# LeoIV/polyaxon

Measured on AMD Instinct MI355X. Metric: HPO trials/hour (whole node) + wall-clock-to-target, ResNet-50 Hyperband sweep, higher is better.
Workload: dtype bf16

## Files before the change

polyaxon_amd/csrc/bn_kernels.hip:

```cpp
#include <hip/hip_runtime.h>

#include "handoff.h"
#include <stdint.h>

#define PLX_API extern "C" __attribute__((visibility("default")))

namespace {

constexpr int kBlock = 256;

struct alignas(16) bf16x8 {
  uint16_t v[8];
};

__device__ __forceinline__ float bf2f(uint16_t b) { return __uint_as_float(((uint32_t)b) << 16); }

__device__ __forceinline__ uint16_t f2bf(float f) {
  return __builtin_bit_cast(uint16_t, (__bf16)f);
}

__device__ __forceinline__ void load8(const bf16x8* p, float* f) {
  const bf16x8 v = *p;
#pragma unroll
  for (int k = 0; k < 8; ++k) f[k] = bf2f(v.v[k]);
// ... 554 lines not shown
inline void reduce_finalize_fwd(hipStream_t stream, const float* part, int nblk, float* l2, unsigned* cnt,
                                const FwdFin& f) {
  const int C = f.C, S = (nblk + kRowsPerSplit - 1) / kRowsPerSplit;
  if (cnt != nullptr) {
    hipLaunchKernelGGL(bn_fwd_reduce_finalize_kernel<kFinNT>, dim3((C + 63) / 64, S), dim3(kFinNT), 0, stream, part, nblk, l2, S,
                       cnt, f);
    return;
  }
  hipLaunchKernelGGL(bn_partial_reduce_kernel<kFinNT>,
                     dim3((C + 63) / 64, S, 2), dim3(kFinNT), 0, stream, part, nblk, C, l2, S);
  hipLaunchKernelGGL(bn_fwd_finalize_kernel<kFinNT>, dim3((C + 63) / 64),
                     dim3(kFinNT), 0, stream, l2, l2 + (int64_t)S * C, S,
                     f.x_row0, C, f.M, f.gamma, f.beta, f.eps, f.momentum, f.running_mean, f.running_var, f.save_mean,
                     f.save_invstd, f.scale, f.bias);
}

inline void reduce_finalize_bwd(hipStream_t stream, const float* part, int nblk, float* l2, unsigned* cnt,
                                const BwdFin& f) {
  const int C = f.C, S = (nblk + kRowsPerSplit - 1) / kRowsPerSplit;
  if (cnt != nullptr) {
    hipLaunchKernelGGL(bn_bwd_reduce_finalize_kernel<kFinNT>, dim3((C + 63) / 64, S), dim3(kFinNT), 0, stream, part, nblk, l2, S,
                       cnt, f);
    return;
  }
  hipLaunchKernelGGL(bn_partial_reduce_kernel<kFinNT>,
                     dim3((C + 63) / 64, S, 2), dim3(kFinNT), 0, stream, part, nblk, C, l2, S);
  hipLaunchKernelGGL(bn_bwd_finalize_kernel<kFinNT>, dim3((C + 63) / 64),
                     dim3(kFinNT), 0, stream, l2, l2 + (int64_t)S * C, S, C,
                     f.M, f.gamma, f.mean, f.invstd, f.dgamma, f.dbeta, f.coef, f.accumulate);
}

struct alignas(8) u8x8 {
  uint8_t v[8];
};

__global__ __launch_bounds__(256) void stem_apply_pool_kernel(const bf16x8* __restrict__ x,
                                                              const float* __restrict__ sb, bf16x8* __restrict__ y,
                                                              u8x8* __restrict__ idx, int N, int H, int W, int G,
                                                              int OH, int OW) {
  const unsigned j = blockIdx.x * 256u + threadIdx.x;
  if (j >= (unsigned)(OW * G)) return;
  const unsigned g = j % (unsigned)G, ow = j / (unsigned)G;
  const int C = G * 8;
  float a[8], b[8];
#pragma unroll
  for (int k = 0; k < 8; ++k) {
    a[k] = sb[g * 8 + k];
    b[k] = sb[C + g * 8 + k];
  }
  for (int row = blockIdx.y; row < N * OH; row += gridDim.y) {
    const int n = row / OH, oh = row - n * OH;
    float best[8];
    uint8_t arg[8];
#pragma unroll
    for (int k = 0; k < 8; ++k) {
      best[k] = -INFINITY;
      arg[k] = 255;
    }
    uint4 q[9];
    bool ok[9];
#pragma unroll
    for (int kh = 0; kh < 3; ++kh) {
      const int ih = oh * 2 - 1 + kh;
      const int ihc = ih < 0 ? 0 : (ih >= H ? H - 1 : ih);
#pragma unroll
      for (int kw = 0; kw < 3; ++kw) {
        const int iw = (int)ow * 2 - 1 + kw;
        const int iwc = iw < 0 ? 0 : (iw >= W ? W - 1 : iw);
        ok[kh * 3 + kw] = ih >= 0 && ih < H && iw >= 0 && iw < W;
        q[kh * 3 + kw] = *(const uint4*)(x + ((size_t)(n * H + ihc) * W + iwc) * G + g);
      }
    }
#pragma unroll
    for (int t9 = 0; t9 < 9; ++t9) {
      const uint32_t qw[4] = {q[t9].x, q[t9].y, q[t9].z, q[t9].w};
#pragma unroll
      for (int k = 0; k < 8; ++k) {
        const float xk = __uint_as_float((k & 1) ? (qw[k >> 1] & 0xffff0000u) : (qw[k >> 1] << 16));
        const float f = (float)(__bf16)fmaxf(fmaf(xk, a[k], b[k]), 0.f);
        if (ok[t9] && (f > best[k] || arg[k] == 255)) {
          best[k] = f;
          arg[k] = (uint8_t)t9;
        }
      }
    }
    bf16x8 o;
    u8x8 m;
#pragma unroll
    for (int k = 0; k < 8; ++k) {
      o.v[k] = f2bf(best[k]);
      m.v[k] = arg[k];
    }
    const size_t t = (size_t)row * OW * G + j;
    y[t] = o;
    idx[t] = m;
  }
}

__device__ __forceinline__ int stem_cover(int i, int O, int* o, int* k) {
  int n = 0;
  if (i & 1) {
    if ((i + 1) >> 1 < O) { o[n] = (i + 1) >> 1; k[n++] = 0; }
    o[n] = (i - 1) >> 1; k[n++] = 2;
  } else if ((i >> 1) < O) {
    o[n] = i >> 1; k[n++] = 1;
  }
  return n;
}

template <bool DX>
__global__ __launch_bounds__(256) void stem_pool_bn_bwd_kernel(const bf16x8* __restrict__ dy, const u8x8* __restrict__ idx,
                                                               const bf16x8* __restrict__ x, const float* __restrict__ sb,
                                                               const float* __restrict__ mean,
                                                               const float* __restrict__ invstd,
                                                               const float* __restrict__ coef, bf16x8* __restrict__ dx,
                                                               float* __restrict__ part, int N, int H, int W, int G,
                                                               int OH, int OW) {
  const int QH = (H + 1) / 2, QW = (W + 1) / 2;
  const unsigned j0 = blockIdx.x * 256u + threadIdx.x;
  const bool active = j0 < (unsigned)(QW * G);
  const unsigned j = active ? j0 : 0u;
  const unsigned g = j % (unsigned)G;
  const int qb = (int)(j / (unsigned)G);
  const int C = G * 8;
  float a[8], b[8], c1[8], c2[8], c3[8], s1[8], s2[8];
#pragma unroll
  for (int k = 0; k < 8; ++k) {
    a[k] = sb[g * 8 + k];
    b[k] = sb[C + g * 8 + k];
    if constexpr (DX) {
      c1[k] = coef[g * 8 + k];
      c2[k] = coef[C + g * 8 + k];
      c3[k] = coef[2 * C + g * 8 + k];
    } else {
      c1[k] = mean[g * 8 + k];
      c2[k] = invstd[g * 8 + k];
      c3[k] = 0.f;
    }
    s1[k] = s2[k] = 0.f;
  }
  for (int row = blockIdx.y; active && row < N * QH; row += gridDim.y) {
    const int n = row / QH, qa = row - n * QH;
    uint2 am[4];
    uint4 d[4], xq[4];
    bool wv[4], pv[4];
#pragma unroll
    for (int p = 0; p < 2; ++p)
#pragma unroll
      for (int q = 0; q < 2; ++q) {
        const int w4 = p * 2 + q, oh = qa + p, ow = qb + q;
        wv[w4] = oh < OH && ow < OW;
        const size_t off = ((size_t)(n * OH + (oh < OH ? oh : OH - 1)) * OW + (ow < OW ? ow : OW - 1)) * G + g;
        am[w4] = *(const uint2*)(idx + off);
        d[w4] = *(const uint4*)(dy + off);
        if (!wv[w4]) am[w4] = make_uint2(0xffffffffu, 0xffffffffu);
        const int ih = 2 * qa + p, iw = 2 * qb + q;
        pv[w4] = ih < H && iw < W;
        xq[w4] = *(const uint4*)(x + ((size_t)(n * H + (ih < H ? ih : H - 1)) * W + (iw < W ? iw : W - 1)) * G + g);
      }
#pragma unroll
    for (int di = 0; di < 2; ++di)
#pragma unroll
      for (int dj = 0; dj < 2; ++dj) {
        const int e = di * 2 + dj;
        const uint32_t xw[4] = {xq[e].x, xq[e].y, xq[e].z, xq[e].w};
        float o[8];
#pragma unroll
        for (int k = 0; k < 8; ++k) {
          float acc = 0.f;
#pragma unroll
          for (int p = 0; p < 2; ++p)
#pragma unroll
            for (int q = 0; q < 2; ++q) {
              const int kh = di + 1 - 2 * p, kw = dj + 1 - 2 * q;
              if (kh < 0 || kw < 0) continue;
              const int w4 = p * 2 + q;
              const uint32_t ab = (k < 4 ? am[w4].x : am[w4].y) >> (8 * (k & 3)) & 0xffu;
              const uint32_t dw = (k >> 1) == 0 ? d[w4].x : (k >> 1) == 1 ? d[w4].y : (k >> 1) == 2 ? d[w4].z : d[w4].w;
              const float dv = __uint_as_float((k & 1) ? (dw & 0xffff0000u) : (dw << 16));
              acc += ab == (uint32_t)(kh * 3 + kw) ? dv : 0.f;
            }
          const float xf = __uint_as_float((k & 1) ? (xw[k >> 1] & 0xffff0000u) : (xw[k >> 1] << 16));
          const float dz = (pv[e] && fmaf(xf, a[k], b[k]) > 0.f) ? (float)(__bf16)acc : 0.f;
          if constexpr (DX) {
            o[k] = fmaf(c1[k], dz, fmaf(c2[k], xf, c3[k]));
          } else {
            s1[k] += dz;
            s2[k] = fmaf(dz, (xf - c1[k]) * c2[k], s2[k]);
          }
        }
        if constexpr (DX) {
          if (pv[e]) store8(dx + ((size_t)(n * H + 2 * qa + di) * W + 2 * qb + dj) * G + g, o);
        }
      }
  }
  if constexpr (!DX) {
    __shared__ float red[256 * 17];
#pragma unroll
    for (int k = 0; k < 8; ++k) {
      red[threadIdx.x * 17 + k] = s1[k];
      red[threadIdx.x * 17 + 8 + k] = s2[k];
    }
    __syncthreads();
    const int nb = gridDim.x * gridDim.y, blk = blockIdx.y * gridDim.x + blockIdx.x;
    for (int e = threadIdx.x; e < G * 16; e += 256) {
      const int gg = e % G, v = e / G;
      float sum = 0.f;
      for (int r = gg; r < 256; r += G) sum += red[r * 17 + v];
      const int c = gg * 8 + (v & 7);
      part[((int64_t)(v < 8 ? 0 : nb) + blk) * C + c] = sum;
    }
  }
}

constexpr int g_stem_bwd_cap = 4096;

inline dim3 stem_bwd_grid(int N, int H, int W, int G, bool dx) {
  const int rows = N * ((H + 1) / 2), cap = dx ? 65535 : g_stem_bwd_cap;
  return dim3((((W + 1) / 2) * G + 255) / 256, rows < cap ? rows : cap);
}

}

PLX_API int64_t plx_bn_workspace(int64_t M, int C) {
  Plan p;
  if (!plan_for(M, C, &p)) return -1;
  return 2 * (int64_t)(p.nblk + p.S) * C;
}

PLX_API int plx_bn_forward(const void* x, const void* res, void* y, int64_t M, int C, const float* gamma,
                           const float* beta, float eps, float momentum, float* running_mean, float* running_var,
                           float* save_mean, float* save_invstd, float* scale_bias ,
                           float* partials , uint8_t* mask ,
                           int relu, const float* res_sb ,
                           unsigned* counters ,
                           hipStream_t stream) {
  Plan p;
  if (!plan_for(M, C, &p) || M < 1) return 1;
  float* psum = partials;
  float* psq = partials + (int64_t)p.nblk * C;
  hipLaunchKernelGGL(bn_stats_kernel, dim3(p.nblk, p.gy), dim3(kBlock), 0, stream, (const bf16x8*)x, M, p.G, p.Gb,
                     p.rows_per_block, psum, psq);
  float* l2 = partials + 2 * (int64_t)p.nblk * C;
  reduce_finalize_fwd(stream, partials, p.nblk, l2, counters,
                      FwdFin{(const uint16_t*)x, C, M, gamma, beta, eps, momentum, running_mean, running_var,
                             save_mean, save_invstd, scale_bias, scale_bias + C});
  const int64_t n_vec = M * p.G;
  if (y != nullptr)
    launch_apply(stream, n_vec, p.G, x, res, y, scale_bias, scale_bias + C, relu, relu ? mask : nullptr, res_sb);
  return (int)hipGetLastError();
}

PLX_API int64_t plx_bn_l2_workspace(int nblk, int C) {
  return 2 * (int64_t)((nblk + kRowsPerSplit - 1) / kRowsPerSplit) * C;
}

PLX_API int plx_bn_forward_from_partials(const void* x, const void* res, void* y, int64_t M, int C,
                                         const float* gamma, const float* beta, float eps, float momentum,
                                         float* running_mean, float* running_var, float* save_mean,
                                         float* save_invstd, float* scale_bias, const float* partials, int nblk,
                                         float* l2, uint8_t* mask, int relu, const float* res_sb,
                                         unsigned* counters, hipStream_t stream) {
  Plan p;
  if (!plan_for(M, C, &p) || M < 1 || nblk < 1) return 1;
  reduce_finalize_fwd(stream, partials, nblk, l2, counters,
                      FwdFin{nullptr, C, M, gamma, beta, eps, momentum, running_mean, running_var, save_mean,
                             save_invstd, scale_bias, scale_bias + C});
  const int64_t n_vec = M * p.G;
  if (y != nullptr)
    launch_apply(stream, n_vec, p.G, x, res, y, scale_bias, scale_bias + C, relu, relu ? mask : nullptr, res_sb);
  return (int)hipGetLastError();
}

PLX_API int plx_bn_apply(const void* x, const void* res, void* y, int64_t M, int C, const float* scale_bias, int relu,
                         hipStream_t stream) {
  Plan p;
  if (!plan_for(M, C, &p)) return 1;
  const int64_t n_vec = M * p.G;
  launch_apply(stream, n_vec, p.G, x, res, y, scale_bias, scale_bias + C, relu, nullptr, nullptr);
  return (int)hipGetLastError();
}

PLX_API int plx_bn_apply_res_relu(const void* x, const void* res, void* y, int64_t M, int C, const float* scale_bias,
                                  uint8_t* mask, const float* res_sb, hipStream_t stream) {
  Plan p;
  if (!plan_for(M, C, &p) || M < 1 || res == nullptr || mask == nullptr) return 1;
  launch_apply(stream, M * p.G, p.G, x, res, y, scale_bias, scale_bias + C, 1, mask, res_sb);
  return (int)hipGetLastError();
}

PLX_API int plx_bn_dx_blocks(int64_t M, int C) {
  Plan p;
  if (!plan_for(M, C, &p)) return -1;
  return apply_grid(M * p.G, p.G);
}

PLX_API int plx_bn_backward(const void* x, const uint8_t* mask, const void* dy, void* dx, void* dres, int64_t M, int C,
                            const float* gamma, const float* save_mean, const float* save_invstd, float* dgamma,
                            float* dbeta, float* coef , float* partials , int relu,
                            int accumulate, const ResBn* resbn , unsigned* counters,
                            hipStream_t stream) {
  Plan p;
  if (!plan_for(M, C, &p) || M < 1 || (relu && mask == nullptr)) return 1;
  if (resbn != nullptr && (dres == nullptr || resbn->part == nullptr)) return 1;
  const ResBn rb = resbn != nullptr ? *resbn : ResBn{};
  float* pa = partials;
  float* pb = partials + (int64_t)p.nblk * C;
  hipLaunchKernelGGL(relu ? bn_bwd_reduce_kernel<true> : bn_bwd_reduce_kernel<false>, dim3(p.nblk, p.gy), dim3(kBlock), 0, stream, (const bf16x8*)x,
                     mask, (const bf16x8*)dy, M, p.G, p.Gb, p.rows_per_block, save_mean, save_invstd,
                     relu, pa, pb);
  float* l2 = partials + 2 * (int64_t)p.nblk * C;
  reduce_finalize_bwd(stream, partials, p.nblk, l2, counters,
                      BwdFin{C, M, gamma, save_mean, save_invstd, dgamma, dbeta, coef, accumulate});
  const int64_t n_vec = M * p.G;
  launch_dx(stream, n_vec, p.G, x, mask, dy, dx, dres, coef, relu, rb);
  return (int)hipGetLastError();
}

PLX_API int plx_bn_backward_from_partials(const void* x, const uint8_t* mask, const void* dy, void* dx, void* dres,
                                          int64_t M, int C, const float* gamma, const float* save_mean,
                                          const float* save_invstd, float* dgamma, float* dbeta, float* coef,
                                          const float* partials, int nblk, float* l2, int relu, int accumulate,
                                          const ResBn* resbn, unsigned* counters, hipStream_t stream) {
  Plan p;
  if (!plan_for(M, C, &p) || M < 1 || nblk < 1 || (relu && mask == nullptr)) return 1;
  if (resbn != nullptr && (dres == nullptr || resbn->part == nullptr)) return 1;
  const ResBn rb = resbn != nullptr ? *resbn : ResBn{};
  reduce_finalize_bwd(stream, partials, nblk, l2, counters,
                      BwdFin{C, M, gamma, save_mean, save_invstd, dgamma, dbeta, coef, accumulate});
  const int64_t n_vec = M * p.G;
  launch_dx(stream, n_vec, p.G, x, mask, dy, dx, dres, coef, relu, rb);
  return (int)hipGetLastError();
}

PLX_API int plx_bn_backward_coef(const void* x, const uint8_t* mask, const void* dy, int64_t M, int C,
                                 const float* gamma, const float* save_mean, const float* save_invstd, float* dgamma,
                                 float* dbeta, float* coef, float* partials, int relu, int accumulate,
                                 unsigned* counters, hipStream_t stream) {
  Plan p;
  if (!plan_for(M, C, &p) || M < 1 || (relu && mask == nullptr)) return 1;
  float* pa = partials;
  float* pb = partials + (int64_t)p.nblk * C;
  hipLaunchKernelGGL(relu ? bn_bwd_reduce_kernel<true> : bn_bwd_reduce_kernel<false>, dim3(p.nblk, p.gy), dim3(kBlock), 0, stream, (const bf16x8*)x,
                     mask, (const bf16x8*)dy, M, p.G, p.Gb, p.rows_per_block, save_mean, save_invstd,
                     relu, pa, pb);
  reduce_finalize_bwd(stream, partials, p.nblk, partials + 2 * (int64_t)p.nblk * C, counters,
                      BwdFin{C, M, gamma, save_mean, save_invstd, dgamma, dbeta, coef, accumulate});
  return (int)hipGetLastError();
}

PLX_API int plx_bn_backward_coef_from_partials(int64_t M, int C, const float* gamma, const float* save_mean,
                                               const float* save_invstd, float* dgamma, float* dbeta, float* coef,
                                               const float* partials, int nblk, float* l2, int accumulate,
                                               unsigned* counters, hipStream_t stream) {
  Plan p;
  if (!plan_for(M, C, &p) || M < 1 || nblk < 1) return 1;
  reduce_finalize_bwd(stream, partials, nblk, l2, counters,
                      BwdFin{C, M, gamma, save_mean, save_invstd, dgamma, dbeta, coef, accumulate});
  return (int)hipGetLastError();
}

PLX_API int plx_stem_bn_pool_forward(const void* x, void* y, void* idx, int N, int H, int W, int C, const float* gamma,
                                     const float* beta, float eps, float momentum, float* running_mean,
                                     float* running_var, float* save_mean, float* save_invstd, float* scale_bias,
                                     float* partials, const float* ext_part, int ext_nblk, unsigned* counters,
                                     hipStream_t stream) {
  const int G = C / 8;
  if (N <= 0 || H <= 0 || W <= 0 || C % 8 || G > 256 || 256 % G) return 1;
  const int rc = ext_part != nullptr
                     ? plx_bn_forward_from_partials(x, nullptr, nullptr, (int64_t)N * H * W, C, gamma, beta, eps,
                                                    momentum, running_mean, running_var, save_mean, save_invstd,
                                                    scale_bias, ext_part, ext_nblk, partials, nullptr, 1, nullptr,
                                                    counters, stream)
                     : plx_bn_forward(x, nullptr, nullptr, (int64_t)N * H * W, C, gamma, beta, eps, momentum,
                                      running_mean, running_var, save_mean, save_invstd, scale_bias, partials, nullptr,
                                      1, nullptr, counters, stream);
  if (rc) return rc;
  const int OH = (H - 1) / 2 + 1, OW = (W - 1) / 2 + 1;
  const int rows = N * OH;
  hipLaunchKernelGGL(stem_apply_pool_kernel, dim3((OW * G + 255) / 256, rows < 65535 ? rows : 65535), dim3(256), 0,
                     stream, (const bf16x8*)x, scale_bias, (bf16x8*)y, (u8x8*)idx, N, H, W, G, OH, OW);
  return (int)hipGetLastError();
}


PLX_API int64_t plx_stem_bn_pool_bwd_workspace(int N, int H, int W, int C) {
  const dim3 g = stem_bwd_grid(N, H, W, C / 8, false);
  const int64_t nblk = (int64_t)g.x * g.y;
  return 2 * (nblk + (nblk + kRowsPerSplit - 1) / kRowsPerSplit) * C;
}

PLX_API int plx_stem_bn_pool_backward(const void* dy, const void* idx, const void* x, void* dx, int N, int H, int W,
                                      int C, const float* gamma, const float* save_mean, const float* save_invstd,
                                      const float* scale_bias, float* dgamma, float* dbeta, float* coef,
                                      float* workspace, int accumulate, unsigned* counters, hipStream_t stream) {
  const int G = C / 8;
  if (N <= 0 || H <= 0 || W <= 0 || C % 8 || G > 256 || 256 % G) return 1;
  const int OH = (H - 1) / 2 + 1, OW = (W - 1) / 2 + 1;
  const dim3 grid = stem_bwd_grid(N, H, W, G, false), grid_dx = stem_bwd_grid(N, H, W, G, true);
  const int nblk = grid.x * grid.y;
  hipLaunchKernelGGL(stem_pool_bn_bwd_kernel<false>, grid, dim3(256), 0, stream, (const bf16x8*)dy, (const u8x8*)idx,
                     (const bf16x8*)x, scale_bias, save_mean, save_invstd, (const float*)nullptr, (bf16x8*)nullptr,
                     workspace, N, H, W, G, OH, OW);
  reduce_finalize_bwd(stream, workspace, nblk, workspace + 2 * (int64_t)nblk * C, counters,
                      BwdFin{C, (int64_t)N * H * W, gamma, save_mean, save_invstd, dgamma, dbeta, coef, accumulate});
  hipLaunchKernelGGL(stem_pool_bn_bwd_kernel<true>, grid_dx, dim3(256), 0, stream, (const bf16x8*)dy, (const u8x8*)idx,
                     (const bf16x8*)x, scale_bias, save_mean, save_invstd, coef, (bf16x8*)dx, (float*)nullptr, N, H,
                     W, G, OH, OW);
  return (int)hipGetLastError();
}
```

polyaxon_amd/ops/bn_fused.py:

```python
from __future__ import annotations

import ctypes

from typing import Optional

import torch

from polyaxon_amd.ops import _native
from polyaxon_amd.ops.conv1x1 import BnLink, PendingApply, fill_pending
from polyaxon_amd.ops.flat import direct_grad


def _stream() -> int:
    return _native.current_stream()


_COUNTERS = {}


def _counters(dev: torch.device):
    key = (dev.index, torch.cuda.current_stream(dev).cuda_stream)
    return _native.cached(_COUNTERS, key, lambda: torch.zeros(64, dtype=torch.int32, device=dev)).data_ptr()


def _cl(t: torch.Tensor) -> torch.Tensor:
    return t if t.is_contiguous(memory_format=torch.channels_last) else t.contiguous(memory_format=torch.channels_last)


def supported(x: torch.Tensor) -> bool:
    if not x.is_cuda or x.dtype != torch.bfloat16 or x.dim() != 4:
        return False
    c = x.shape[1]
    g = c // 8
    return c % 8 == 0 and g > 0 and (g & (g - 1)) == 0 and x.numel() > 0


class _BNAct(torch.autograd.Function):
    @staticmethod
    def forward(ctx, x, weight, bias, running_mean, running_var, residual, momentum, eps, relu, ext=None, box=None,
                link=None, rlink=None, defer=False, dxsink=None, pend=None):
        lib = _native.lib("plx_bn")
        ctx.dxsink = dxsink if x.is_contiguous(memory_format=torch.channels_last) else None
        x = _cl(x)
        n, c, h, w = x.shape
        m = n * h * w
        ws = _native.size("plx_bn", "plx_bn_workspace", m, c)
        if ws < 0:
            raise RuntimeError("unsupported channel count for fused BN")
        f32 = dict(dtype=torch.float32, device=x.device)
        defer = bool(defer) and not relu and residual is None and link is not None
        y = None if defer else torch.empty_like(x, memory_format=torch.channels_last)
        holder, pend = pend, pend is not None and relu and residual is not None and not defer
        yp = y.data_ptr() if (y is not None and not pend) else None
        stats = torch.empty(4 * c, **f32)
        res_sb = None
        if residual is not None:
            rl = getattr(residual, "_plx_bn_link", None)
            if rl is not None and rl.affine is not None and getattr(residual, "_plx_deferred", False):
                res_sb = rl.affine
        res = _cl(residual) if residual is not None else None
        rsp = res_sb.data_ptr() if res_sb is not None else None
        rm = running_mean.data_ptr() if running_mean is not None else None
        rv = running_var.data_ptr() if running_var is not None else None
        mask = torch.empty(m * c // 8, dtype=torch.uint8, device=x.device) if relu else None
        mp = mask.data_ptr() if mask is not None else None
        if ext is not None:
            part, nblk = ext
            l2 = torch.empty(_native.size("plx_bn", "plx_bn_l2_workspace", nblk, c), **f32)
            rc = lib.plx_bn_forward_from_partials(
                x.data_ptr(), res.data_ptr() if res is not None else None, yp, m, c, weight.data_ptr(),
                bias.data_ptr(), float(eps), float(momentum), rm, rv, stats.data_ptr(), stats[c:].data_ptr(),
                stats[2 * c:].data_ptr(), part.data_ptr(), nblk, l2.data_ptr(), mp, int(relu), rsp,
                _counters(x.device), _stream())
            _native.check(rc, "plx_bn_forward_from_partials")
        else:
            partials = torch.empty(ws, **f32)
            rc = lib.plx_bn_forward(
                x.data_ptr(), res.data_ptr() if res is not None else None, yp, m, c,
                weight.data_ptr(), bias.data_ptr(), float(eps), float(momentum), rm, rv,
                stats.data_ptr(), stats[c:].data_ptr(), stats[2 * c:].data_ptr(), partials.data_ptr(), mp, int(relu),
                rsp, _counters(x.device), _stream())
            _native.check(rc, "plx_bn_forward")
        ctx.save_for_backward(x, mask, weight, stats)
        ctx.pending = PendingApply(x, res, stats[2 * c:], res_sb, mask, y) if pend else None
        if pend:
            holder.append(ctx.pending)
        ctx.relu = relu
        ctx.has_res = residual is not None
        ctx.box = box if (box is not None and box.armed and residual is not None) else None
        if ctx.box is not None:
            ctx.box.expect = True
        ctx.ws = ws
        gw, gb = direct_grad(weight), direct_grad(bias)
        ctx.direct = (gw, gb) if (gw is not None and gb is not None) else None
        ctx.link = link
        if link is not None:
            link.x, link.mask, link.mean, link.invstd = x, mask, stats[:c], stats[c:2 * c]
            if defer:
                link.affine = stats[2 * c:]
        ctx.rlink = rlink if (rlink is not None and residual is not None and rlink.x is not None
                              and rlink.x.shape == x.shape and ctx.box is None) else None
        if defer:
            return x.view_as(x)
        return y

    @staticmethod
    def backward(ctx, dy):
        lib = _native.lib("plx_bn")
        x, mask, weight, stats = ctx.saved_tensors
        if ctx.pending is not None:
            ctx.pending.check_done()
        n, c, h, w = x.shape
        m = n * h * w
        dy = _cl(dy)
        if dy.dtype != torch.bfloat16:
            dy = dy.to(torch.bfloat16)
        f32 = dict(dtype=torch.float32, device=x.device)
        dx = torch.empty_like(x, memory_format=torch.channels_last)
        masked_box = ctx.box is not None and ctx.relu and mask is not None
        dres = (torch.empty_like(x, memory_format=torch.channels_last)
                if ctx.has_res and not masked_box else None)
        if ctx.direct is not None:
            dg_ptr, db_ptr, acc = ctx.direct[0].data_ptr(), ctx.direct[1].data_ptr(), 1
            dgb = None
        else:
            dgb = torch.empty(2 * c, **f32)
            dg_ptr, db_ptr, acc = dgb.data_ptr(), dgb[c:].data_ptr(), 0
        coef = torch.empty(3 * c, **f32)
        part, nblk = ctx.link.take() if ctx.link is not None else (None, 0)
        if ctx.dxsink is not None and dres is None:
            if part is not None:
                l2 = torch.empty(_native.size("plx_bn", "plx_bn_l2_workspace", nblk, c), **f32)
                rc = lib.plx_bn_backward_coef_from_partials(
                    m, c, weight.data_ptr(), stats.data_ptr(), stats[c:].data_ptr(), dg_ptr, db_ptr, coef.data_ptr(),
                    part.data_ptr(), nblk, l2.data_ptr(), acc, _counters(x.device), _stream())
                _native.check(rc, "plx_bn_backward_coef_from_partials")
            else:
                partials = torch.empty(ctx.ws, **f32)
                rc = lib.plx_bn_backward_coef(
                    x.data_ptr(), mask.data_ptr() if mask is not None else None, dy.data_ptr(), m, c,
                    weight.data_ptr(), stats.data_ptr(), stats[c:].data_ptr(), dg_ptr, db_ptr, coef.data_ptr(),
                    partials.data_ptr(), int(ctx.relu), acc, _counters(x.device), _stream())
                _native.check(rc, "plx_bn_backward_coef")
            ctx.dxsink.put(dy, x, mask if ctx.relu else None, coef, dx)
            if ctx.box is not None:
                ctx.box.put_masked(dy, mask)
            dgamma = dgb[:c] if dgb is not None else None
            dbeta = dgb[c:] if dgb is not None else None
            return dx, dgamma, dbeta, None, None, None, None, None, None, None, None, None, None, None, None, None
        rb = None
        if ctx.rlink is not None and dres is not None:
            rl = ctx.rlink
            nblk2 = _native.size("plx_bn", "plx_bn_dx_blocks", m, c)
            rl.part = torch.empty(2 * nblk2 * c, **f32)
            rl.nblk = nblk2
            rb = _native.ResBnArgs(rl.x.data_ptr(), rl.mask.data_ptr() if rl.mask is not None else None,
                                   rl.mean.data_ptr(), rl.invstd.data_ptr(), rl.part.data_ptr())
        rbp = ctypes.addressof(rb) if rb is not None else None
        if part is not None:
            l2 = torch.empty(_native.size("plx_bn", "plx_bn_l2_workspace", nblk, c), **f32)
            rc = lib.plx_bn_backward_from_partials(
                x.data_ptr(), mask.data_ptr() if mask is not None else None, dy.data_ptr(), dx.data_ptr(),
                dres.data_ptr() if dres is not None else None, m, c, weight.data_ptr(), stats.data_ptr(),
                stats[c:].data_ptr(), dg_ptr, db_ptr, coef.data_ptr(), part.data_ptr(), nblk, l2.data_ptr(),
                int(ctx.relu), acc, rbp, _counters(x.device), _stream())
            _native.check(rc, "plx_bn_backward_from_partials")
        else:
            partials = torch.empty(ctx.ws, **f32)
            rc = lib.plx_bn_backward(
                x.data_ptr(), mask.data_ptr() if mask is not None else None, dy.data_ptr(), dx.data_ptr(),
                dres.data_ptr() if dres is not None else None, m, c, weight.data_ptr(), stats.data_ptr(),
                stats[c:].data_ptr(), dg_ptr, db_ptr, coef.data_ptr(), partials.data_ptr(), int(ctx.relu), acc,
                rbp, _counters(x.device), _stream())
            _native.check(rc, "plx_bn_backward")
        if ctx.box is not None:
            if masked_box:
                ctx.box.put_masked(dy, mask)
            else:
                ctx.box.put(dres)
            dres = None
        dgamma = dgb[:c] if dgb is not None else None
        dbeta = dgb[c:] if dgb is not None else None
        return dx, dgamma, dbeta, None, None, dres, None, None, None, None, None, None, None, None, None, None


class _Materialize(torch.autograd.Function):

    @staticmethod
    def forward(ctx, t, sb):
        c = t.shape[1]
        return (t.float() * sb[:c].view(1, c, 1, 1) + sb[c:].view(1, c, 1, 1)).to(t.dtype).contiguous(
            memory_format=torch.channels_last)

    @staticmethod
    def backward(ctx, g):
        return g, None


def materialize(t: Optional[torch.Tensor]) -> Optional[torch.Tensor]:
    if t is None:
        return t
    fill_pending(t)
    if not getattr(t, "_plx_deferred", False):
        return t
    return _Materialize.apply(t, t._plx_bn_link.affine)


def bn_act(x: torch.Tensor, weight: torch.Tensor, bias: torch.Tensor, running_mean: Optional[torch.Tensor],
           running_var: Optional[torch.Tensor], training: bool, momentum: float, eps: float,
           residual: Optional[torch.Tensor], act: bool, ext_stats=None, residual_grad_box=None,
           residual_link: bool = False, defer_apply: bool = False, dx_sink=None,
           defer_res_relu: bool = False) -> torch.Tensor:
    fill_pending(residual)
    if residual is not None and residual.dtype != x.dtype:
        residual = residual.to(x.dtype)
    if training:
        link = BnLink()
        rlink = getattr(residual, "_plx_bn_link", None) if (residual_link and residual is not None) else None
        defer = bool(defer_apply) and not act and residual is None
        pend = [] if (defer_res_relu and act and residual is not None) else None
        y = _BNAct.apply(x, weight, bias, running_mean, running_var, residual, momentum, eps, act, ext_stats,
                         residual_grad_box, link, rlink, defer, dx_sink, pend)
        y._plx_bn_link = link
        if defer:
            y._plx_deferred = True
        if pend:
            y._plx_pending = pend[0]
        return y
    residual = materialize(residual)
    lib = _native.lib("plx_bn")
    x = _cl(x)
    n, c, h, w = x.shape
    inv = torch.rsqrt(running_var.float() + eps)
    scale = weight.float() * inv
    sb = torch.cat([scale, bias.float() - running_mean.float() * scale]).contiguous()
    y = torch.empty_like(x, memory_format=torch.channels_last)
    res = _cl(residual) if residual is not None else None
    rc = lib.plx_bn_apply(x.data_ptr(), res.data_ptr() if res is not None else None, y.data_ptr(), n * h * w, c,
                          sb.data_ptr(), int(act), _stream())
    _native.check(rc, "plx_bn_apply")
    return y
```

polyaxon_amd/ops/conv1x1.py:

```python
from __future__ import annotations

import ctypes
import os
from typing import Dict

import torch
import torch.nn as nn
import torch.nn.functional as F

from polyaxon_amd.ops import _native, side_stream, wcache
from polyaxon_amd.ops.flat import direct_grad

_ZERO: Dict[int, torch.Tensor] = {}
_CUS: Dict[int, int] = {}

_BN_DX_FUSED = os.environ.get("PLX_BN_DX_FUSED", "1") != "0"


def set_bn_dx_fused(on: bool) -> bool:
    global _BN_DX_FUSED
    prev, _BN_DX_FUSED = _BN_DX_FUSED, bool(on)
    return prev


_BN_APPLY_FUSED = os.environ.get("PLX_BN_APPLY_FUSED", "1") != "0"


def set_bn_apply_fused(on: bool) -> bool:
    global _BN_APPLY_FUSED
    prev, _BN_APPLY_FUSED = _BN_APPLY_FUSED, bool(on)
    return prev


def bn_apply_fused() -> bool:
    return _BN_APPLY_FUSED


def _zero_page(dev: torch.device) -> torch.Tensor:
    idx = dev.index if dev.index is not None else torch.cuda.current_device()
    return _native.cached(_ZERO, idx, lambda: torch.zeros(256, dtype=torch.bfloat16, device=dev))


def _num_cus(dev: torch.device) -> int:
    idx = dev.index if dev.index is not None else torch.cuda.current_device()
    if idx not in _CUS:
        _CUS[idx] = torch.cuda.get_device_properties(idx).multi_processor_count
    return _CUS[idx]


def _stream() -> int:
    return _native.current_stream()


def nt_stats_rows(n: int) -> int:
    return _native.size("plx_conv", "plx_gemm_nt_rows_per_block", n)


def gemm_nt(a: torch.Tensor, b: torch.Tensor, out: torch.Tensor = None, stats: torch.Tensor = None,
            add: torch.Tensor = None, bnr: "_native.BnBwdArgs" = None, add_mask: torch.Tensor = None) -> torch.Tensor:
    m, k = a.shape
    n = b.shape[0]
    if out is None:
        out = torch.empty(m, n, dtype=torch.bfloat16, device=a.device)
    assert a.stride(1) == 1 and b.stride(1) == 1 and out.stride(1) == 1 and b.shape[1] == k
    assert a.data_ptr() % 16 == 0 and b.data_ptr() % 16 == 0 and out.data_ptr() % 16 == 0
    if stats is not None:
        nblk = -(-m // nt_stats_rows(n))
        assert stats.dtype == torch.float32 and stats.is_contiguous() and stats.numel() >= 2 * nblk * n
    if add is not None:
        assert add.shape == (m, n) and add.stride(1) == 1 and add.dtype == torch.bfloat16 and add.data_ptr() % 16 == 0
    if add_mask is not None:
        assert add is not None and add.stride(0) == n and add_mask.dtype == torch.uint8 and add_mask.numel() == m * n // 8
    rc = _native.lib("plx_conv").plx_gemm_nt(a.data_ptr(), b.data_ptr(), out.data_ptr(), m, n, k, a.stride(0),
                                             b.stride(0), out.stride(0), _zero_page(a.device).data_ptr(),
                                             stats.data_ptr() if stats is not None else None,
                                             add.data_ptr() if add is not None else None,
                                             add.stride(0) if add is not None else 0,
                                             add_mask.data_ptr() if add_mask is not None else None,
                                             ctypes.addressof(bnr) if bnr is not None else None, _stream())
    _native.check(rc, "plx_gemm_nt")
    return out


def gemm_nt_bndx(g: torch.Tensor, x: torch.Tensor, mask: torch.Tensor, coef: torch.Tensor, dy: torch.Tensor,
                 b: torch.Tensor, out: torch.Tensor = None, add: torch.Tensor = None,
                 bnr: "_native.BnBwdArgs" = None, add_mask: torch.Tensor = None) -> torch.Tensor:
    m, k = g.shape
    n = b.shape[0]
    if out is None:
        out = torch.empty(m, n, dtype=torch.bfloat16, device=g.device)
    for t in (g, x, dy):
        assert t.shape == (m, k) and t.dtype == torch.bfloat16 and t.stride() == (k, 1) and t.data_ptr() % 16 == 0
    assert b.stride(1) == 1 and out.stride(1) == 1 and b.shape[1] == k and b.dtype == torch.bfloat16
    assert b.data_ptr() % 16 == 0 and out.data_ptr() % 16 == 0
    assert coef.dtype == torch.float32 and coef.is_contiguous() and coef.numel() == 3 * k
    if mask is not None:
        assert mask.dtype == torch.uint8 and mask.numel() == m * k // 8
    if add is not None:
        assert add.shape == (m, n) and add.stride(1) == 1 and add.dtype == torch.bfloat16 and add.data_ptr() % 16 == 0
    if add_mask is not None:
        assert add is not None and add.stride(0) == n and add_mask.dtype == torch.uint8 and add_mask.numel() == m * n // 8
    rc = _native.lib("plx_conv").plx_gemm_nt_bndx(g.data_ptr(), x.data_ptr(),
                                                  mask.data_ptr() if mask is not None else None, coef.data_ptr(),
                                                  dy.data_ptr(), b.data_ptr(), out.data_ptr(), m, n, k, b.stride(0),
                                                  out.stride(0), add.data_ptr() if add is not None else None,
                                                  add.stride(0) if add is not None else 0,
                                                  add_mask.data_ptr() if add_mask is not None else None,
                                                  ctypes.addressof(bnr) if bnr is not None else None, _stream())
    _native.check(rc, "plx_gemm_nt_bndx")
    return out


def gemm_nt_bnapply(x: torch.Tensor, res: torch.Tensor, sb: torch.Tensor, rsb, out_a: torch.Tensor, mask: torch.Tensor,
                    b: torch.Tensor, out: torch.Tensor = None, stats: torch.Tensor = None) -> torch.Tensor:
    m, k = x.shape
    n = b.shape[0]
    if out is None:
        out = torch.empty(m, n, dtype=torch.bfloat16, device=x.device)
    for t in (x, res, out_a):
        assert t.shape == (m, k) and t.dtype == torch.bfloat16 and t.stride() == (k, 1) and t.data_ptr() % 16 == 0
    assert b.stride(1) == 1 and out.stride(1) == 1 and b.shape[1] == k and b.dtype == torch.bfloat16
    assert b.data_ptr() % 16 == 0 and out.data_ptr() % 16 == 0
    assert mask.dtype == torch.uint8 and mask.is_contiguous() and mask.numel() >= m * k // 8
    for c in (sb, rsb):
        assert c is None or (c.dtype == torch.float32 and c.is_contiguous() and c.numel() == 2 * k
                             and c.data_ptr() % 16 == 0)
    assert sb is not None
    if stats is not None:
        nblk = -(-m // nt_stats_rows(n))
        assert stats.dtype == torch.float32 and stats.is_contiguous() and stats.numel() >= 2 * nblk * n
    rc = _native.lib("plx_conv").plx_gemm_nt_bnapply(x.data_ptr(), res.data_ptr(), sb.data_ptr(),
                                                     rsb.data_ptr() if rsb is not None else None, out_a.data_ptr(),
                                                     mask.data_ptr(), b.data_ptr(), out.data_ptr(), m, n, k,
                                                     b.stride(0), out.stride(0),
                                                     stats.data_ptr() if stats is not None else None, _stream())
    _native.check(rc, "plx_gemm_nt_bnapply")
    return out


def gemm_tn(a: torch.Tensor, b: torch.Tensor, out: torch.Tensor = None, accumulate: bool = False) -> torch.Tensor:
    m, n1 = a.shape
    n2 = b.shape[1]
    if out is None:
        out = torch.empty(n1, n2, dtype=torch.float32, device=a.device)
        accumulate = False
    assert a.stride(1) == 1 and b.stride(1) == 1 and out.stride(1) == 1 and b.shape[0] == m
    assert a.data_ptr() % 16 == 0 and b.data_ptr() % 16 == 0 and out.data_ptr() % 16 == 0
    lib = _native.lib("plx_conv")
    cus = _num_cus(a.device)
    ws = torch.empty(_native.size("plx_conv", "plx_gemm_tn_workspace", m, n1, n2, cus), dtype=torch.float32,
                     device=a.device)
    rc = lib.plx_gemm_tn(a.data_ptr(), b.data_ptr(), out.data_ptr(), ws.data_ptr(), m, n1, n2, a.stride(0),
                         b.stride(0), out.stride(0), _zero_page(a.device).data_ptr(), cus, int(accumulate),
                         _stream())
    _native.check(rc, "plx_gemm_tn")
    return out


def weight_prep(w: torch.Tensor):
    cout, cin = w.shape[0], w.shape[1]
    wb = torch.empty(cout, cin, dtype=torch.bfloat16, device=w.device)
    wt = torch.empty(cin, cout, dtype=torch.bfloat16, device=w.device)
    w32 = w.reshape(cout, cin)
    if w32.dtype != torch.float32 or not w32.is_contiguous():
        w32 = w32.float().contiguous()
    rc = _native.lib("plx_conv").plx_weight_prep(w32.data_ptr(), wb.data_ptr(), wt.data_ptr(), cout, cin, _stream())
    _native.check(rc, "plx_weight_prep")
    return wb, wt


class GradMailbox:

    __slots__ = ("armed", "grad", "mask", "expect", "s2k1")

    def __init__(self):
        self.armed = False
        self.grad = None
        self.mask = None
        self.expect = False
        self.s2k1 = False

    def put(self, g: torch.Tensor) -> None:
        if self.grad is not None:
            g = self._dense() + g
        self.grad, self.mask = g, None

    def put_masked(self, g: torch.Tensor, mask: torch.Tensor) -> None:
        if self.grad is not None:
            self.put(unpack_relu_mask(g, mask))
            return
        self.grad, self.mask = g, mask

    def _dense(self) -> torch.Tensor:
        return self.grad if self.mask is None else unpack_relu_mask(self.grad, self.mask)

    def take(self):
        g, m = self.grad, self.mask
        self.grad = self.mask = None
        if g is None and self.expect:
            raise RuntimeError("GradMailbox: the deferred gradient did not arrive before its consumer's backward")
        return g, m


def unpack_relu_mask(g: torch.Tensor, mask: torch.Tensor) -> torch.Tensor:
    bits = (mask.view(-1, 1) >> torch.arange(8, device=mask.device, dtype=torch.uint8)) & 1
    n, c, h, w = g.shape
    keep = bits.view(n, h, w, c).permute(0, 3, 1, 2).to(g.dtype)
    return (g * keep).contiguous(memory_format=torch.channels_last)


class DxSink:

    __slots__ = ("payload",)

    def __init__(self):
        self.payload = None

    def put(self, g: torch.Tensor, x: torch.Tensor, mask, coef: torch.Tensor, dx: torch.Tensor) -> None:
        self.payload = (g, x, mask, coef, dx)

    def take(self):
        p, self.payload = self.payload, None
        return p


def dx_sink_for(x: torch.Tensor, weight: torch.Tensor):
    if not _BN_DX_FUSED or not (torch.is_grad_enabled() and x.requires_grad):
        return None
    cout, cin = weight.shape[0], weight.shape[1]
    return DxSink() if (cout >= 2 * cin and cin <= 128) else None


class PendingApply:

    __slots__ = ("x", "res", "sb", "rsb", "mask", "out", "state")

    def __init__(self, x, res, sb, rsb, mask, out):
        self.x, self.res, self.sb, self.rsb, self.mask, self.out = x, res, sb, rsb, mask, out
        self.state = "pending"

    @property
    def pending(self) -> bool:
        return self.state == "pending"

    def take(self) -> "PendingApply":
        if self.state != "pending":
            raise RuntimeError("PendingApply: the deferred BatchNorm output was already " + self.state
                               + "; a second consumer cannot take it")
        self.state = "taken"
        return self

    def fill(self) -> None:
        if self.state != "pending":
            return
        n, c, h, w = self.x.shape
        rc = _native.lib("plx_bn").plx_bn_apply_res_relu(
            self.x.data_ptr(), self.res.data_ptr(), self.out.data_ptr(), n * h * w, c, self.sb.data_ptr(),
            self.mask.data_ptr(), self.rsb.data_ptr() if self.rsb is not None else None, _stream())
        _native.check(rc, "plx_bn_apply_res_relu")
        self.state = "filled"
        self.release()

    def release(self) -> None:
        self.x = self.res = self.sb = self.rsb = self.mask = self.out = None

    def check_done(self) -> None:
        if self.state == "pending":
            raise RuntimeError("PendingApply: the BatchNorm's deferred output (and its ReLU mask) was never filled: "
                               "no consumer took it and nothing materialised it before the backward")


def fill_pending(t):
    p = getattr(t, "_plx_pending", None) if t is not None else None
    if p is not None:
        p.fill()
    return t


def bn_apply_sink_ok(cin: int, cout: int) -> bool:
    return _BN_APPLY_FUSED and cin >= 2 * cout and cout <= 128


class BnLink:

    __slots__ = ("x", "mask", "mean", "invstd", "part", "nblk", "_args", "affine", "split")

    def __init__(self, x=None, mask=None, mean=None, invstd=None):
        self.x, self.mask, self.mean, self.invstd = x, mask, mean, invstd
        self.affine = None
        self.part = None
        self.nblk = 0
        self._args = None
        self.split = 0

    def _args_for(self, nblk_total: int, blk_off: int) -> "_native.BnBwdArgs":
        return _native.BnBwdArgs(self.x.data_ptr(), self.mask.data_ptr() if self.mask is not None else None,
                                 self.mean.data_ptr(), self.invstd.data_ptr(), self.part.data_ptr(), nblk_total,
                                 blk_off)

    def request(self, nblk: int) -> "_native.BnBwdArgs":
        c = self.x.shape[1]
        self.part = torch.empty(2 * nblk * c, dtype=torch.float32, device=self.x.device)
        self.nblk, self.split = nblk, 0
        self._args = self._args_for(nblk, 0)
        return self._args

    def request_split(self, nblk1: int, nblk2: int) -> "_native.BnBwdArgs":
        n, c, h, w = self.x.shape
        self.part = torch.empty(2 * (nblk1 + nblk2) * c, dtype=torch.float32, device=self.x.device)
        self.nblk, self.split = nblk1 + nblk2, nblk1
        a = self._args_for(nblk1 + nblk2, 0)
        a.skip_h, a.skip_w = h, w
        self._args = a
        return a

    def request_rest(self) -> "_native.BnBwdArgs":
        a = self._args_for(self.nblk, self.split)
        self.split = 0
        self._args = a
        return a

    def take(self):
        part, nblk = self.part, self.nblk
        if self.split:
            part, nblk = None, 0
        self.part, self._args, self.split = None, None, 0
        return part, nblk


def _rows(t: torch.Tensor) -> torch.Tensor:
    n, c, h, w = t.shape
    return t.permute(0, 2, 3, 1).reshape(n * h * w, c)


def bn_link_of(x: torch.Tensor, want: bool):
    link = getattr(x, "_plx_bn_link", None) if want else None
    return link if (link is not None and link.x is not None and link.x.shape == x.shape) else None


class _Conv1x1(torch.autograd.Function):
    @staticmethod
    def forward(ctx, x, weight, stats, box, sink, link, dxsink=None, pend=None):
        if pend is not None and (x.data_ptr() != pend.out.data_ptr() or x.shape != pend.out.shape
                                 or x.dtype != torch.bfloat16
                                 or not x.is_contiguous(memory_format=torch.channels_last)):
            raise RuntimeError("PendingApply: the convolution's input is not the deferred BatchNorm output")
        x = x.to(torch.bfloat16).contiguous(memory_format=torch.channels_last)
        ctx.box = box
        ctx.dxsink = dxsink
        ctx.sink = sink if (sink is not None and sink.armed) else None
        if ctx.sink is not None:
            ctx.sink.expect = True
        ctx.link = link if (sink is None or sink.armed) else None
        ctx.wgrad = direct_grad(weight)
        n, cin, h, w = x.shape
        cout = weight.shape[0]
        wb, wt = wcache.lookup(weight) or weight_prep(weight)
        y = torch.empty((n, cout, h, w), dtype=torch.bfloat16, device=x.device, memory_format=torch.channels_last)
        if pend is not None:
            gemm_nt_bnapply(_rows(pend.x), _rows(pend.res), pend.sb, pend.rsb, _rows(x), pend.mask, wb, _rows(y), stats)
            pend.release()
        else:
            gemm_nt(_rows(x), wb, _rows(y), stats)
        ctx.save_for_backward(x, wt)
        ctx.wshape = weight.shape
        ctx.wdtype = weight.dtype
        return y

    @staticmethod
    def backward(ctx, dy):
        x, wt = ctx.saved_tensors
        n, cin, h, w = x.shape
        fused = ctx.dxsink.take() if ctx.dxsink is not None else None
        if fused is not None and (dy.data_ptr() != fused[4].data_ptr() or dy.shape != fused[4].shape
                                  or dy.dtype != torch.bfloat16 or not ctx.needs_input_grad[0]):
            raise RuntimeError("DxSink: the BatchNorm's deferred input gradient was replaced before the convolution's "
                               "backward could fill it")
        dy = dy.to(torch.bfloat16).contiguous(memory_format=torch.channels_last)
        dx = dw = None
        extra, extra_mask = ctx.box.take() if ctx.box is not None else (None, None)
        if ctx.needs_input_grad[0]:
            dx = torch.empty_like(x, memory_format=torch.channels_last)
            if extra is not None and (extra.dtype != torch.bfloat16
                                      or not extra.is_contiguous(memory_format=torch.channels_last)):
                if extra_mask is not None:
                    extra, extra_mask = unpack_relu_mask(extra, extra_mask), None
                extra = extra.to(torch.bfloat16).contiguous(memory_format=torch.channels_last)
            bnr = None
            rows = nt_stats_rows(cin)
            if ctx.link is not None and ctx.sink is None and (ctx.box is None or extra is not None):
                bnr = ctx.link.request(-(-(n * h * w) // rows))
            elif ctx.link is not None and ctx.sink is not None and ctx.sink.s2k1 and extra is None:
                bnr = ctx.link.request_split(-(-(n * h * w) // rows), -(-(n * ((h + 1) // 2) * ((w + 1) // 2)) // rows))
            if fused is not None:
                g, bx, bmask, coef, _ = fused
                gemm_nt_bndx(_rows(g), _rows(bx), bmask, coef, _rows(dy), wt, _rows(dx),
                             add=_rows(extra) if extra is not None else None, bnr=bnr, add_mask=extra_mask)
            else:
                gemm_nt(_rows(dy), wt, _rows(dx), add=_rows(extra) if extra is not None else None, bnr=bnr,
                        add_mask=extra_mask)
            if ctx.sink is not None:
                ctx.sink.put(dx)
                dx = None
        if ctx.needs_input_grad[1]:
            cout = ctx.wshape[0]
            if ctx.wgrad is not None:
                slot = ctx.wgrad.as_strided((cout, cin), (cin, 1))
                side_stream.run(lambda: gemm_tn(_rows(dy), _rows(x), out=slot, accumulate=True), (dy, x), x.device)
            else:
                dw = gemm_tn(_rows(dy), _rows(x)).view(ctx.wshape).to(ctx.wdtype)
        return dx, dw, None, None, None, None, None, None


def _bf16_context(x: torch.Tensor) -> bool:
    if x.dtype == torch.bfloat16:
        return True
    return torch.is_autocast_enabled("cuda") and torch.get_autocast_dtype("cuda") == torch.bfloat16


def supported(x: torch.Tensor, conv: nn.Conv2d) -> bool:
    return (x.is_cuda and x.dim() == 4 and _bf16_context(x) and conv.kernel_size == (1, 1) and conv.stride == (1, 1)
            and conv.padding == (0, 0) and conv.groups == 1 and conv.bias is None
            and conv.in_channels % 64 == 0 and conv.out_channels % 64 == 0 and x.numel() > 0)


def conv1x1(x: torch.Tensor, weight: torch.Tensor, with_stats: bool = False,
            grad_box: "GradMailbox" = None, grad_sink: "GradMailbox" = None, bn_link: bool = False) -> torch.Tensor:
    stats = None
    if with_stats:
        n, _, h, w = x.shape
        m, cout = n * h * w, weight.shape[0]
        nblk = -(-m // nt_stats_rows(cout))
        stats = torch.empty(2 * nblk * cout, dtype=torch.float32, device=x.device)
    if grad_box is not None:
        grad_box.armed = True
    dxsink = dx_sink_for(x, weight)
    pend = getattr(x, "_plx_pending", None)
    if pend is not None and pend.pending:
        n, cin, h, w = x.shape
        if bn_apply_sink_ok(cin, weight.shape[0]) and n * h * w * cin < (1 << 30):
            pend = pend.take()
        else:
            pend.fill()
            pend = None
    else:
        pend = None
    y = _Conv1x1.apply(x, weight, stats, grad_box, grad_sink, bn_link_of(x, bn_link), dxsink, pend)
    if stats is not None:
        y._plx_channel_stats = (stats, nblk)
    if dxsink is not None:
        y._plx_dx_sink = dxsink
    return y


class Conv1x1(nn.Conv2d):

    def __init__(self, in_ch: int, out_ch: int, stride: int = 1, native: bool = True, bn_stats: bool = True):
        super().__init__(in_ch, out_ch, 1, stride=stride, bias=False)
        self.native = native
        self.bn_stats = bn_stats

    def forward(self, x: torch.Tensor, grad_box: GradMailbox = None, grad_sink: GradMailbox = None,
                bn_link: bool = False) -> torch.Tensor:
        if self.native and supported(x, self):
            return conv1x1(x, self.weight, with_stats=self.bn_stats and self.training, grad_box=grad_box,
                           grad_sink=grad_sink, bn_link=bn_link)
        return F.conv2d(fill_pending(x), self.weight, None, self.stride)
```

Baseline: 12820.

## Pass unmasked residual gradient with ReLU mask to linked residual BatchNorm

When a fused BN+residual+ReLU backward feeds a linked residual BatchNorm, the residual gradient is no longer written to its own buffer. The upstream dy is handed over together with the ReLU mask, and the downstream BN backward applies the mask itself as a relu gradient. This removes a full activation-sized write and read of dres. In exchange it adds cross-op state and validation that dy was not replaced, and it relaxes the native check that required a dres pointer.

```diff
diff --git a/polyaxon_amd/csrc/bn_kernels.hip b/polyaxon_amd/csrc/bn_kernels.hip
--- a/polyaxon_amd/csrc/bn_kernels.hip
+++ b/polyaxon_amd/csrc/bn_kernels.hip
@@ -880,7 +880,7 @@
                             hipStream_t stream) {
   Plan p;
   if (!plan_for(M, C, &p) || M < 1 || (relu && mask == nullptr)) return 1;
-  if (resbn != nullptr && (dres == nullptr || resbn->part == nullptr)) return 1;
+  if (resbn != nullptr && resbn->part == nullptr) return 1;
   const ResBn rb = resbn != nullptr ? *resbn : ResBn{};
   float* pa = partials;
   float* pb = partials + (int64_t)p.nblk * C;
@@ -902,7 +902,7 @@
                                           const ResBn* resbn, unsigned* counters, hipStream_t stream) {
   Plan p;
   if (!plan_for(M, C, &p) || M < 1 || nblk < 1 || (relu && mask == nullptr)) return 1;
-  if (resbn != nullptr && (dres == nullptr || resbn->part == nullptr)) return 1;
+  if (resbn != nullptr && resbn->part == nullptr) return 1;
   const ResBn rb = resbn != nullptr ? *resbn : ResBn{};
   reduce_finalize_bwd(stream, partials, nblk, l2, counters,
                       BwdFin{C, M, gamma, save_mean, save_invstd, dgamma, dbeta, coef, accumulate});
diff --git a/polyaxon_amd/ops/bn_fused.py b/polyaxon_amd/ops/bn_fused.py
--- a/polyaxon_amd/ops/bn_fused.py
+++ b/polyaxon_amd/ops/bn_fused.py
@@ -1,6 +1,7 @@
 from __future__ import annotations
 
 import ctypes
+import os
 
 from typing import Optional
 
@@ -13,6 +14,15 @@
 
 def _stream() -> int:
     return _native.current_stream()
+
+
+_BN_DRES_MASKED = os.environ.get("PLX_BN_DRES_MASKED", "1") != "0"
+
+
+def set_bn_dres_masked(on: bool) -> bool:
+    global _BN_DRES_MASKED
+    prev, _BN_DRES_MASKED = _BN_DRES_MASKED, bool(on)
+    return prev
 
 
 _COUNTERS = {}
@@ -112,14 +122,23 @@
             ctx.pending.check_done()
         n, c, h, w = x.shape
         m = n * h * w
+        lm = ctx.link.take_masked() if ctx.link is not None else None
+        if lm is not None and (dy.data_ptr() != lm[0].data_ptr() or dy.shape != lm[0].shape
+                               or dy.dtype != torch.bfloat16 or ctx.relu
+                               or not dy.is_contiguous(memory_format=torch.channels_last)):
+            raise RuntimeError("BnLink: the masked residual gradient was replaced before the BatchNorm's backward "
+                               "could apply its mask")
         dy = _cl(dy)
         if dy.dtype != torch.bfloat16:
             dy = dy.to(torch.bfloat16)
+        gmask, grelu = (lm[1], True) if lm is not None else (mask, ctx.relu)
         f32 = dict(dtype=torch.float32, device=x.device)
         dx = torch.empty_like(x, memory_format=torch.channels_last)
         masked_box = ctx.box is not None and ctx.relu and mask is not None
+        masked_link = (_BN_DRES_MASKED and ctx.rlink is not None and ctx.has_res and ctx.relu and mask is not None
+                       and not masked_box and ctx.rlink.mask is None)
         dres = (torch.empty_like(x, memory_format=torch.channels_last)
-                if ctx.has_res and not masked_box else None)
+                if ctx.has_res and not masked_box and not masked_link else None)
         if ctx.direct is not None:
             dg_ptr, db_ptr, acc = ctx.direct[0].data_ptr(), ctx.direct[1].data_ptr(), 1
             dgb = None
@@ -128,7 +147,7 @@
             dg_ptr, db_ptr, acc = dgb.data_ptr(), dgb[c:].data_ptr(), 0
         coef = torch.empty(3 * c, **f32)
         part, nblk = ctx.link.take() if ctx.link is not None else (None, 0)
-        if ctx.dxsink is not None and dres is None:
+        if ctx.dxsink is not None and dres is None and not masked_link:
             if part is not None:
                 l2 = torch.empty(_native.size("plx_bn", "plx_bn_l2_workspace", nblk, c), **f32)
                 rc = lib.plx_bn_backward_coef_from_partials(
@@ -138,18 +157,18 @@
             else:
                 partials = torch.empty(ctx.ws, **f32)
                 rc = lib.plx_bn_backward_coef(
-                    x.data_ptr(), mask.data_ptr() if mask is not None else None, dy.data_ptr(), m, c,
+                    x.data_ptr(), gmask.data_ptr() if gmask is not None else None, dy.data_ptr(), m, c,
                     weight.data_ptr(), stats.data_ptr(), stats[c:].data_ptr(), dg_ptr, db_ptr, coef.data_ptr(),
-                    partials.data_ptr(), int(ctx.relu), acc, _counters(x.device), _stream())
+                    partials.data_ptr(), int(grelu), acc, _counters(x.device), _stream())
                 _native.check(rc, "plx_bn_backward_coef")
-            ctx.dxsink.put(dy, x, mask if ctx.relu else None, coef, dx)
+            ctx.dxsink.put(dy, x, gmask if grelu else None, coef, dx)
             if ctx.box is not None:
                 ctx.box.put_masked(dy, mask)
             dgamma = dgb[:c] if dgb is not None else None
             dbeta = dgb[c:] if dgb is not None else None
             return dx, dgamma, dbeta, None, None, None, None, None, None, None, None, None, None, None, None, None
         rb = None
-        if ctx.rlink is not None and dres is not None:
+        if ctx.rlink is not None and (dres is not None or masked_link):
             rl = ctx.rlink
             nblk2 = _native.size("plx_bn", "plx_bn_dx_blocks", m, c)
             rl.part = torch.empty(2 * nblk2 * c, **f32)
@@ -160,19 +179,22 @@
         if part is not None:
             l2 = torch.empty(_native.size("plx_bn", "plx_bn_l2_workspace", nblk, c), **f32)
             rc = lib.plx_bn_backward_from_partials(
-                x.data_ptr(), mask.data_ptr() if mask is not None else None, dy.data_ptr(), dx.data_ptr(),
+                x.data_ptr(), gmask.data_ptr() if gmask is not None else None, dy.data_ptr(), dx.data_ptr(),
                 dres.data_ptr() if dres is not None else None, m, c, weight.data_ptr(), stats.data_ptr(),
                 stats[c:].data_ptr(), dg_ptr, db_ptr, coef.data_ptr(), part.data_ptr(), nblk, l2.data_ptr(),
-                int(ctx.relu), acc, rbp, _counters(x.device), _stream())
+                int(grelu), acc, rbp, _counters(x.device), _stream())
             _native.check(rc, "plx_bn_backward_from_partials")
         else:
             partials = torch.empty(ctx.ws, **f32)
             rc = lib.plx_bn_backward(
-                x.data_ptr(), mask.data_ptr() if mask is not None else None, dy.data_ptr(), dx.data_ptr(),
+                x.data_ptr(), gmask.data_ptr() if gmask is not None else None, dy.data_ptr(), dx.data_ptr(),
                 dres.data_ptr() if dres is not None else None, m, c, weight.data_ptr(), stats.data_ptr(),
-                stats[c:].data_ptr(), dg_ptr, db_ptr, coef.data_ptr(), partials.data_ptr(), int(ctx.relu), acc,
+                stats[c:].data_ptr(), dg_ptr, db_ptr, coef.data_ptr(), partials.data_ptr(), int(grelu), acc,
                 rbp, _counters(x.device), _stream())
             _native.check(rc, "plx_bn_backward")
+        if masked_link:
+            ctx.rlink.put_masked(dy, mask)
+            dres = dy
         if ctx.box is not None:
             if masked_box:
                 ctx.box.put_masked(dy, mask)
diff --git a/polyaxon_amd/ops/conv1x1.py b/polyaxon_amd/ops/conv1x1.py
--- a/polyaxon_amd/ops/conv1x1.py
+++ b/polyaxon_amd/ops/conv1x1.py
@@ -283,7 +283,7 @@
 
 class BnLink:
 
-    __slots__ = ("x", "mask", "mean", "invstd", "part", "nblk", "_args", "affine", "split")
+    __slots__ = ("x", "mask", "mean", "invstd", "part", "nblk", "_args", "affine", "split", "masked")
 
     def __init__(self, x=None, mask=None, mean=None, invstd=None):
         self.x, self.mask, self.mean, self.invstd = x, mask, mean, invstd
@@ -292,6 +292,7 @@
         self.nblk = 0
         self._args = None
         self.split = 0
+        self.masked = None
 
     def _args_for(self, nblk_total: int, blk_off: int) -> "_native.BnBwdArgs":
         return _native.BnBwdArgs(self.x.data_ptr(), self.mask.data_ptr() if self.mask is not None else None,
@@ -319,6 +320,13 @@
         self.split = 0
         self._args = a
         return a
+
+    def put_masked(self, g: torch.Tensor, mask: torch.Tensor) -> None:
+        self.masked = (g, mask)
+
+    def take_masked(self):
+        p, self.masked = self.masked, None
+        return p
 
     def take(self):
         part, nblk = self.part, self.nblk
```

Measured after the change: 12900, median of 6. No clear change (+0.6%).
